# zfw1226/active_tracking_rl

Hardware: AMD Instinct MI355X
Metric: env steps/sec, Track2D-BlockPartialPZR-v0 @4096 envs, 1/2/4/8 GPU (higher is better)
Workload: dtype u8 map bits / f64 reward -> f32 obs+reward; policy fp32

## Files before the change

### active_tracking_rl_amd/csrc/gemm_tn_hip.hip

```cpp
#include <hip/hip_runtime.h>
#include <stdint.h>
#include <stdlib.h>

#include "../../include/atr_policy.h"

namespace atr {

typedef float f32x16 __attribute__((ext_vector_type(16)));

#ifndef ATR_TN_DIRECT
#define ATR_TN_DIRECT 1
#endif
#ifndef ATR_TN_PROBE
#define ATR_TN_PROBE 0
#endif
constexpr int kTile = 128, kLd = 128;
constexpr int kGemmThreads = 256;
constexpr long long kSmallK = 20 * 1024 + 1;
constexpr int tn_wg_per_cu(int kc) { return kc == 32 ? 2 : kc == 24 ? 3 : 4; }
static thread_local int g_tn_corun = 0;
static int tn_kc(long long K)
{
    static const int forced = getenv("ATR_GEMM_TN_KC") ? atoi(getenv("ATR_GEMM_TN_KC")) : 0;
    if (forced == 16 || forced == 32) return forced;
    if (g_tn_corun) return 16;
    return K < kSmallK ? 16 : 32;
}
static int tn_wg_per_cu_now(int kc) { return g_tn_corun ? 1 : tn_wg_per_cu(kc); }
constexpr unsigned kCorunLdsPad = 50000;

template <int kKC> struct GemmLds { float a[2][kKC][kLd]; float b[2][kKC][kLd]; };

constexpr int kMaxProblems = 8;

struct TnProblem {
    const float *x1, *x2;
    float *partial;
    float *cs_partial;
    const float *row_scale;
    float *c;
    float *cs_out0, *cs_out1;
    long long rs_shift;
    long long ld1, ld2;
    int M, N;
    int tile_begin;
    int red_begin;
};

struct TnGroup {
    TnProblem p[kMaxProblems];
    long long K;
    int count, slices, chunks_per_slice, tiles_total;
    int red_blocks;
};

#if ATR_TN_PROBE
__device__ unsigned long long g_tn_stamps[8192 * 4];
#endif

template <int kKC, bool kMixed>
__global__ __launch_bounds__(kGemmThreads, tn_wg_per_cu(kKC)) void k_gemm_tn(const TnGroup g)
{
    __shared__ __attribute__((aligned(16))) GemmLds<kKC> s;
    const int tid = (int)threadIdx.x, l = tid & 63, wave = tid >> 6;
#if ATR_TN_PROBE
    const unsigned long long st_rt = wall_clock64(), st_cy = __builtin_readcyclecounter();
#endif
    const int wm = wave >> 1, wn = wave & 1;
    const int i = (int)blockIdx.x, xcd = i & 7, in_xcd = i >> 3;
    const int slice = xcd + 8 * (in_xcd / g.tiles_total), tg = in_xcd % g.tiles_total;
    if (slice >= g.slices) return;
    int q = 0;
#pragma unroll
    for (int j = 1; j < kMaxProblems; j++)
        if (j < g.count && tg >= g.p[j].tile_begin) q = j;
    const float *__restrict__ x1 = g.p[q].x1, *__restrict__ x2 = g.p[q].x2;
    float *__restrict__ partial = g.p[q].partial, *__restrict__ colsum_partial = g.p[q].cs_partial;
    const float *__restrict__ row_scale = g.p[q].row_scale;
    const long long rs_shift = g.p[q].rs_shift, K = g.K;
    const int M = g.p[q].M, N = g.p[q].N, tile = tg - g.p[q].tile_begin, chunks_per_slice = g.chunks_per_slice;
    const int tiles_n = N / kTile;
    const int m0 = (tile / tiles_n) * kTile, n0 = (tile % tiles_n) * kTile;
    const long long k_begin = (long long)slice * chunks_per_slice * kKC;
    long long k_end = k_begin + (long long)chunks_per_slice * kKC;
    if (k_end > K) k_end = K;
    const int r = tid >> 5, c4 = tid & 31;
    const float4 *g1 = reinterpret_cast<const float4 *>(x1 + m0 + c4 * 4), *g2 = reinterpret_cast<const float4 *>(x2 + n0 + c4 * 4);
    const long long ldm = g.p[q].ld1 / 4, ldn = g.p[q].ld2 / 4;
    float4 ra0, ra1, rb0, rb1, ra2, ra3, rb2, rb3;
    float rs0 = 1.f, rs1 = 1.f, rs2 = 1.f, rs3 = 1.f;
    const bool do_colsum = colsum_partial != nullptr && n0 == 0;
    float cs = 0.f;
    const float4 zero4 = make_float4(0.f, 0.f, 0.f, 0.f);
#define GEMM_TN_FETCH(k0_)                                                     \
    {                                                                          \
        const long long ka_ = (k0_) + r, kb_ = (k0_) + r + 8, kc_ = (k0_) + r + 16, kd_ = (k0_) + r + 24;  \
        ra0 = zero4; ra1 = zero4; rb0 = zero4; rb1 = zero4; ra2 = zero4; ra3 = zero4; rb2 = zero4; rb3 = zero4; \
        if (ka_ < k_end) { ra0 = g1[ka_ * ldm]; rb0 = g2[ka_ * ldn]; }         \
        if (kb_ < k_end) { ra1 = g1[kb_ * ldm]; rb1 = g2[kb_ * ldn]; }         \
        if (kKC >= 24 && kc_ < k_end) { ra2 = g1[kc_ * ldm]; rb2 = g2[kc_ * ldn]; }         \
        if (kKC == 32 && kd_ < k_end) { ra3 = g1[kd_ * ldm]; rb3 = g2[kd_ * ldn]; }         \
        if (row_scale) {           \
            rs0 = 1.f; rs1 = 1.f; rs2 = 1.f; rs3 = 1.f;                       \
            if (ka_ >= rs_shift && ka_ < k_end) rs0 = row_scale[ka_ - rs_shift];                                       \
            if (kb_ >= rs_shift && kb_ < k_end) rs1 = row_scale[kb_ - rs_shift];                                       \
            if (kKC >= 24 && kc_ >= rs_shift && kc_ < k_end) rs2 = row_scale[kc_ - rs_shift];                         \
            if (kKC == 32 && kd_ >= rs_shift && kd_ < k_end) rs3 = row_scale[kd_ - rs_shift];                         \
        }                                                                      \
    }
#define GEMM_TN_STAGE(buf_)                                                    \
    {                                                                          \
        if (row_scale) {                                                       \
            ra0.x *= rs0; ra0.y *= rs0; ra0.z *= rs0; ra0.w *= rs0; ra1.x *= rs1; ra1.y *= rs1; ra1.z *= rs1; ra1.w *= rs1; \
            ra2.x *= rs2; ra2.y *= rs2; ra2.z *= rs2; ra2.w *= rs2; ra3.x *= rs3; ra3.y *= rs3; ra3.z *= rs3; ra3.w *= rs3; \
        }                                                                      \
        *reinterpret_cast<float4 *>(&s.a[buf_][r][c4 * 4]) = ra0;              \
        *reinterpret_cast<float4 *>(&s.a[buf_][r + 8][c4 * 4]) = ra1;          \
        *reinterpret_cast<float4 *>(&s.b[buf_][r][c4 * 4]) = rb0;              \
        *reinterpret_cast<float4 *>(&s.b[buf_][r + 8][c4 * 4]) = rb1;          \
        if (kKC >= 24) {                                                       \
        *reinterpret_cast<float4 *>(&s.a[buf_][(r + 16) % kKC][c4 * 4]) = ra2;         \
        *reinterpret_cast<float4 *>(&s.b[buf_][(r + 16) % kKC][c4 * 4]) = rb2;         \
        }                                                                      \
        if (kKC == 32) {                                                       \
        *reinterpret_cast<float4 *>(&s.a[buf_][(r + 24) % kKC][c4 * 4]) = ra3;         \
        *reinterpret_cast<float4 *>(&s.b[buf_][(r + 24) % kKC][c4 * 4]) = rb3;         \
        }                                                                      \
    }
    f32x16 acc00, acc01, acc10, acc11;
#pragma unroll
    for (int q = 0; q < 16; q++) { acc00[q] = 0.f; acc01[q] = 0.f; acc10[q] = 0.f; acc11[q] = 0.f; }
    const int kr = l >> 5, col = l & 31;
    auto compute = [&](int buf) {
        const float *pa = &s.a[buf][kr][wm * 64 + col], *pb = &s.b[buf][kr][wn * 64 + col];
        float a0 = pa[0], a1 = pa[32], b0 = pb[0], b1 = pb[32];
#pragma unroll
        for (int kp = 0; kp < kKC / 2; kp++) {
            float na0 = 0.f, na1 = 0.f, nb0 = 0.f, nb1 = 0.f;
            if (kp + 1 < kKC / 2) {
                na0 = pa[(kp + 1) * 2 * kLd]; na1 = pa[(kp + 1) * 2 * kLd + 32];
                nb0 = pb[(kp + 1) * 2 * kLd]; nb1 = pb[(kp + 1) * 2 * kLd + 32];
            }
            __builtin_amdgcn_sched_barrier(0);
            acc00 = __builtin_amdgcn_mfma_f32_32x32x2f32(a0, b0, acc00, 0, 0, 0);
            acc01 = __builtin_amdgcn_mfma_f32_32x32x2f32(a0, b1, acc01, 0, 0, 0);
            acc10 = __builtin_amdgcn_mfma_f32_32x32x2f32(a1, b0, acc10, 0, 0, 0);
            acc11 = __builtin_amdgcn_mfma_f32_32x32x2f32(a1, b1, acc11, 0, 0, 0);
            a0 = na0; a1 = na1; b0 = nb0; b1 = nb1;
        }
        if (do_colsum) {
            const float *pc = &s.a[buf][(tid >> 7) * (kKC / 2)][tid & 127];
#pragma unroll
            for (int q = 0; q < kKC / 2; q++) cs += pc[q * kLd];
        }
    };
    const bool direct = !kMixed || (kKC == 32 && ATR_TN_DIRECT && row_scale == nullptr && k_end > k_begin && (k_end - k_begin) % kKC == 0);
    if (direct) {
        auto dma = [&](long long k0, int buf) {
#pragma unroll
            for (int j = 0; j < kKC / 8; j++) {
                const long long kk = k0 + r + 8 * j;
                __builtin_amdgcn_global_load_lds((const __attribute__((address_space(1))) void *)(g1 + kk * ldm),
                                                 (__attribute__((address_space(3))) void *)(&s.a[buf][2 * wave + 8 * j][0]), 16, 0, 0);
                __builtin_amdgcn_global_load_lds((const __attribute__((address_space(1))) void *)(g2 + kk * ldn),
                                                 (__attribute__((address_space(3))) void *)(&s.b[buf][2 * wave + 8 * j][0]), 16, 0, 0);
            }
        };
        if (k_begin < k_end) dma(k_begin, 0);
        __builtin_amdgcn_s_waitcnt(0x0F70);
        __syncthreads();
        int buf = 0;
        for (long long k0 = k_begin; k0 < k_end; k0 += kKC, buf ^= 1) {
            if (k0 + kKC < k_end) dma(k0 + kKC, buf ^ 1);
            compute(buf);
            __builtin_amdgcn_s_waitcnt(0x0F70);
            __syncthreads();
        }
    } else if (kMixed) {
        GEMM_TN_FETCH(k_begin);
        GEMM_TN_STAGE(0);
        __syncthreads();
        int buf = 0;
        for (long long k0 = k_begin; k0 < k_end; k0 += kKC, buf ^= 1) {
            const bool more = k0 + kKC < k_end;
            if (more) GEMM_TN_FETCH(k0 + kKC);
            compute(buf);
            if (more) GEMM_TN_STAGE(buf ^ 1);
            __syncthreads();
        }
    }
    if (do_colsum) {
        float *red = &s.a[0][0][0];
        if (tid >= 128) red[tid - 128] = cs;
        __syncthreads();
        if (tid < 128) colsum_partial[(size_t)slice * M + m0 + tid] = cs + red[tid];
    }
#undef GEMM_TN_FETCH
#undef GEMM_TN_STAGE
    float *out = partial + (size_t)slice * M * N;
    auto store = [&](const f32x16 &acc, int mt, int nt) {
#pragma unroll
        for (int q = 0; q < 16; q++) {
            const int row = (q & 3) + 8 * (q >> 2) + 4 * kr;
            __builtin_nontemporal_store(acc[q], &out[(size_t)(m0 + wm * 64 + mt * 32 + row) * N + n0 + wn * 64 + nt * 32 + col]);
        }
    };
    store(acc00, 0, 0); store(acc01, 0, 1); store(acc10, 1, 0); store(acc11, 1, 1);
#if ATR_TN_PROBE
    if (tid == 0 && blockIdx.x < 8192) {
        unsigned long long *o = &g_tn_stamps[(size_t)blockIdx.x * 4];
        o[0] = st_rt; o[1] = wall_clock64(); o[2] = __builtin_readcyclecounter() - st_cy;
        o[3] = (unsigned long long)__builtin_amdgcn_s_getreg(63492) | ((unsigned long long)__builtin_amdgcn_s_getreg(63508) << 32);
    }
#endif
}

__global__ __launch_bounds__(256) void k_gemm_tn_reduce(const TnGroup g)
{
    const int b = (int)blockIdx.x;
    if (b < g.red_blocks) {
        int q = 0;
#pragma unroll
        for (int j = 1; j < kMaxProblems; j++)
            if (j < g.count && b >= g.p[j].red_begin) q = j;
        const long long mn = (long long)g.p[q].M * g.p[q].N;
        const long long i = ((long long)(b - g.p[q].red_begin) * 256 + threadIdx.x) * 4;
        if (i >= mn) return;
        const float *__restrict__ partial = g.p[q].partial;
        float4 acc = *reinterpret_cast<const float4 *>(partial + i);
#pragma unroll 8
        for (int z = 1; z < g.slices; z++) {
            const float4 t = *reinterpret_cast<const float4 *>(partial + (size_t)z * mn + i);
            acc.x += t.x; acc.y += t.y; acc.z += t.z; acc.w += t.w;
        }
        *reinterpret_cast<float4 *>(g.p[q].c + i) = acc;
        return;
    }
    int cb = b - g.red_blocks;
    for (int q = 0; q < g.count; q++) {
        if (!g.p[q].cs_partial) continue;
        const int nb = g.p[q].M / 4;
        if (cb >= nb) { cb -= nb; continue; }
        const int col = cb * 4 + (int)(threadIdx.x >> 6), lane = (int)(threadIdx.x & 63u), M = g.p[q].M;
        const float *__restrict__ partial = g.p[q].cs_partial;
        float acc = 0.f;
        for (int z = lane; z < g.slices; z += 64) acc += partial[(size_t)z * M + col];
        for (int m = 32; m >= 1; m >>= 1) acc += __shfl_xor(acc, m, 64);
        if (lane == 0) {
            if (g.p[q].cs_out0) g.p[q].cs_out0[col] = acc;
            if (g.p[q].cs_out1) g.p[q].cs_out1[col] = acc;
        }
        return;
    }
}

struct TnPlan { int slices, chunks_per_slice; };

static TnPlan gemm_tn_plan(long long K, int tiles)
{
    const int kKC = tn_kc(K), kWgPerCu = tn_wg_per_cu_now(kKC);
    const long long chunks = (K + kKC - 1) / kKC;
    const double eff_pair = 0.85, eff_solo = 0.6;
    int best = 8;
    double best_cost = 1e30;
    static const int forced = getenv("ATR_GEMM_TN_SLICES") ? atoi(getenv("ATR_GEMM_TN_SLICES")) : 0;
    for (int s = 8; s <= 512; s += 8) {
        if (s > chunks && s > 8) break;
        const long long cps = (chunks + s - 1) / s, wgs = (long long)tiles * s;
        const double rows = (double)cps * kKC + 64.0;
        const long long round = 256 * kWgPerCu;
        const long long full = wgs / round, rem = wgs - full * round;
        double cost = (double)full * kWgPerCu * rows / eff_pair;
        if (rem > 256) cost += (double)((rem + 255) / 256) * rows / eff_pair;
        else if (rem > 0) cost += rows / eff_solo;
        if (cost < best_cost - 1e-9) { best_cost = cost; best = s; }
    }
    if (forced >= 8 && forced % 8 == 0 && forced <= chunks) best = forced;
    TnPlan p;
    p.chunks_per_slice = (int)((chunks + best - 1) / best);
    p.slices = best;
    return p;
}

static int group_tiles(const atr_gemm_tn_problem *pr, int count)
{
    int tiles = 0;
    for (int q = 0; q < count; q++) {
        if (!pr[q].x1 || !pr[q].x2 || !pr[q].c || pr[q].M <= 0 || pr[q].N <= 0 || pr[q].M % kTile || pr[q].N % kTile) return -1;
        if ((pr[q].ld1 && (pr[q].ld1 < pr[q].M || pr[q].ld1 % 4)) || (pr[q].ld2 && (pr[q].ld2 < pr[q].N || pr[q].ld2 % 4))) return -1;
        tiles += (pr[q].M / kTile) * (pr[q].N / kTile);
    }
    return tiles;
}

}

using namespace atr;

#if ATR_TN_PROBE
extern "C" int atr_tn_stamps(unsigned long long *host, int wgs)
{
    return (int)hipMemcpyFromSymbol(host, HIP_SYMBOL(g_tn_stamps), (size_t)wgs * 4 * sizeof(unsigned long long));
}
#endif

extern "C" long long atr_gemm_tn_grouped_workspace_floats(const atr_gemm_tn_problem *problems, int count, long long K)
{
    if (!problems || count < 1 || count > kMaxProblems || K <= 0) return -1;
    const int tiles = group_tiles(problems, count);
    if (tiles < 0) return -1;
    const int s = gemm_tn_plan(K, tiles).slices;
    long long total = 0;
    for (int q = 0; q < count; q++) total += (long long)s * problems[q].M * problems[q].N + (long long)s * problems[q].M;
    return total;
}

extern "C" int atr_gemm_tn_grouped(const atr_gemm_tn_problem *problems, int count, long long K, float *workspace, void *stream)
{
    if (!problems || !workspace || count < 1 || count > kMaxProblems || K <= 0) return -1;
    const int tiles = group_tiles(problems, count);
    if (tiles < 0) return -1;
    TnGroup g;
    const TnPlan plan = gemm_tn_plan(K, tiles);
    g.slices = plan.slices; g.chunks_per_slice = plan.chunks_per_slice;
    g.K = K; g.count = count; g.tiles_total = tiles;
    float *ws = workspace;
    int tile_begin = 0, red_begin = 0, cs_blocks = 0;
    for (int q = 0; q < kMaxProblems; q++) {
        TnProblem &d = g.p[q];
        if (q >= count) { d = g.p[0]; d.tile_begin = 1 << 30; d.red_begin = 1 << 30; continue; }
        const atr_gemm_tn_problem &p = problems[q];
        const long long mn = (long long)p.M * p.N;
        d.x1 = p.x1; d.x2 = p.x2; d.c = p.c; d.row_scale = p.row_scale; d.rs_shift = p.row_scale_shift; d.M = p.M; d.N = p.N;
        d.ld1 = p.ld1 ? p.ld1 : p.M; d.ld2 = p.ld2 ? p.ld2 : p.N;
        d.cs_out0 = p.colsum0; d.cs_out1 = p.colsum1;
        d.partial = ws; ws += (size_t)g.slices * mn;
        const bool cs = p.colsum0 || p.colsum1;
        d.cs_partial = cs ? ws : nullptr;
        if (cs) { ws += (size_t)g.slices * p.M; cs_blocks += p.M / 4; }
        d.tile_begin = tile_begin; tile_begin += (p.M / kTile) * (p.N / kTile);
        d.red_begin = red_begin; red_begin += (int)((mn / 4 + 255) / 256);
    }
    g.red_blocks = red_begin;
    hipStream_t st = (hipStream_t)stream;
    const dim3 grid((unsigned)(g.slices * tiles)), block(kGemmThreads);
    const int kc = tn_kc(K);
    static const unsigned forced_pad = getenv("ATR_GEMM_TN_LDS_PAD") ? (unsigned)atoi(getenv("ATR_GEMM_TN_LDS_PAD")) : 0u;
    const unsigned lds_pad = forced_pad ? forced_pad : (g_tn_corun && kc == 16 ? kCorunLdsPad : 0u);
    static bool attr_set = false;
    if (lds_pad && !attr_set) {
        const int lim = 96 * 1024;
        if (hipFuncSetAttribute((const void *)k_gemm_tn<16, false>, hipFuncAttributeMaxDynamicSharedMemorySize, lim) != hipSuccess ||
            hipFuncSetAttribute((const void *)k_gemm_tn<16, true>, hipFuncAttributeMaxDynamicSharedMemorySize, lim) != hipSuccess ||
            hipFuncSetAttribute((const void *)k_gemm_tn<32, false>, hipFuncAttributeMaxDynamicSharedMemorySize, lim) != hipSuccess ||
            hipFuncSetAttribute((const void *)k_gemm_tn<32, true>, hipFuncAttributeMaxDynamicSharedMemorySize, lim) != hipSuccess)
            return -2;
        attr_set = true;
    }
    bool all_direct = ATR_TN_DIRECT && K % kc == 0;
    for (int q = 0; q < count; q++) all_direct = all_direct && problems[q].row_scale == nullptr;
    if (kc == 16) {
        if (all_direct) hipLaunchKernelGGL((k_gemm_tn<16, false>), grid, block, lds_pad, st, g);
        else hipLaunchKernelGGL((k_gemm_tn<16, true>), grid, block, lds_pad, st, g);
    } else {
        if (all_direct) hipLaunchKernelGGL((k_gemm_tn<32, false>), grid, block, lds_pad, st, g);
        else hipLaunchKernelGGL((k_gemm_tn<32, true>), grid, block, lds_pad, st, g);
    }
    hipLaunchKernelGGL(k_gemm_tn_reduce, dim3((unsigned)(red_begin + cs_blocks)), dim3(256), 0, st, g);
    return hipGetLastError() == hipSuccess ? 0 : -2;
}

extern "C" int atr_gemm_tn_set_corun(int on)
{
    const int was = g_tn_corun;
    g_tn_corun = on ? 1 : 0;
    return was;
}

extern "C" long long atr_gemm_tn_workspace_floats(long long K, int M, int N)
{
    atr_gemm_tn_problem p = {};
    float dummy = 0.f;
    p.x1 = p.x2 = &dummy; p.c = &dummy; p.M = M; p.N = N; p.colsum0 = &dummy;
    return atr_gemm_tn_grouped_workspace_floats(&p, 1, K);
}

extern "C" int atr_gemm_tn(const float *x1, const float *x2, float *c, float *workspace, long long K, int M, int N,
                           const float *row_scale, float *colsum, void *stream)
{
    atr_gemm_tn_problem p = {};
    p.x1 = x1; p.x2 = x2; p.c = c; p.M = M; p.N = N; p.row_scale = row_scale; p.row_scale_shift = 0; p.colsum0 = colsum;
    return atr_gemm_tn_grouped(&p, 1, K, workspace, stream);
}
```

### active_tracking_rl_amd/fused.py

```python
import ctypes as C
import json
import os
import re
import sys

import torch

from . import vec_env

_lib = None


class ActStepArgs(C.Structure):
    _fields_ = [("ig", C.c_void_p * 2), ("hg", C.c_void_p * 2), ("bias", C.c_void_p * 2), ("c_prev", C.c_void_p * 2),
                ("h_out", C.c_void_p * 2), ("c_out", C.c_void_p * 2), ("acts", C.c_void_p * 2),
                ("actor_w", C.c_void_p * 2), ("actor_b", C.c_void_p * 2), ("emb", C.c_void_p), ("done_prev", C.c_void_p),
                ("actions_out", C.c_void_p), ("counter", C.c_void_p), ("seed", C.c_ulonglong), ("ordinal", C.c_uint),
                ("A", C.c_int), ("N", C.c_int), ("R", C.c_int), ("hm_out", C.c_void_p * 2), ("hm_ld", C.c_longlong)]


class CoopStepArgs(C.Structure):
    _fields_ = [("y", C.c_void_p * 2), ("fc_w", C.c_void_p * 2), ("fc_b", C.c_void_p * 2), ("w_cat", C.c_void_p * 2),
                ("ldy", C.c_longlong * 2), ("kfc", C.c_int * 2), ("fh", C.c_void_p), ("gates", C.c_void_p),
                ("fh_pstride", C.c_longlong), ("fh_ld", C.c_longlong), ("F", C.c_int), ("workgroups", C.c_int),
# ... 1224 lines not shown


@torch.no_grad()
def gae_returns(rewards, values, notdone, gamma, tau):
    T, N, A = rewards.shape[0], rewards.shape[1], rewards.shape[2]
    rewards, values, notdone = rewards.contiguous(), values.contiguous(), notdone.contiguous()
    ret, gae = torch.empty_like(rewards), torch.empty_like(rewards)
    lib().atr_gae_returns(_p(rewards), _p(values), _p(notdone), float(gamma), float(tau), _p(ret), _p(gae),
                          T, N, A, _stream(rewards))
    return ret, gae


def _col_stride(t):
    return t.shape[-2] if t.shape[-1] == 1 else t.shape[-1]


@torch.no_grad()
def heads_values(h, critic, values, off):
    h = h.contiguous()
    rows, R = h.shape
    A = _col_stride(values)
    lib().atr_heads_values(_p(h), _p(critic.weight), _p(critic.bias), _p(values), rows, R, A, off, _stream(h))


@torch.no_grad()
def heads_values2(hs, critics, values):
    h0, h1 = hs[0].contiguous(), hs[1].contiguous()
    rows, R = h0.shape
    assert h1.shape == h0.shape
    A = _col_stride(values)
    lib().atr_heads_values2(_p(h0), _p(critics[0].weight), _p(critics[0].bias), 0, _p(h1), _p(critics[1].weight),
                            _p(critics[1].bias), 1, _p(values), rows, R, A, _stream(h0))


def _act_layout(actions, rows):
    if actions.dim() == 2 and actions.stride(1) == 1 and actions.shape[0] * actions.shape[1] == rows:
        return actions, actions.shape[1], actions.stride(0)
    a = actions.reshape(rows).contiguous()
    return a, rows, 0


def _head_grads(dh, gs, A, R, has_aux):
    o = (A + 2) * R
    dwa, dwc, dwx = gs[:A * R].view(A, R), gs[A * R:(A + 1) * R].view(1, R), gs[(A + 1) * R:o].view(1, R)
    dba, dbc, dbx = gs[o:o + A], gs[o + A:o + A + 1], gs[o + A + 1:o + A + 2]
    return [dh, dwa, dba, dwc, dbc, dwx if has_aux else None, dbx if has_aux else None]


class _HeadsLossPair(torch.autograd.Function):

    @staticmethod
    def forward(ctx, cfg, *t):
        L = lib()
        arr = (HeadsLossArgs * 2)()
        hs, keep = [], []
        for p in range(2):
            h, wa, ba, wc, bc, waux, baux = t[7 * p:7 * p + 7]
            c = cfg[p]
            h = h.contiguous()
            rows, R = h.shape
            A = wa.shape[0]
            rec = (A + 2) * R + (A + 2) + 4
            dh = torch.empty_like(h)
            gs = torch.empty(rec + 1, dtype=torch.float32, device=h.device)
            ws = torch.empty(L.atr_heads_workspace_floats(rows, R, A), dtype=torch.float32, device=h.device)
            acts, act_n, act_ts = _act_layout(c["actions"], rows)
            ret = c["ret"]
            a = arr[p]
            a.h, a.actions, a.act_n, a.act_tstride = h.data_ptr(), acts.data_ptr(), act_n, act_ts
            a.ret, a.gae, a.val = ret.data_ptr(), c["gae"].data_ptr(), c["val"].data_ptr()
            a.stride = _col_stride(ret)
            a.off = c["off"]
            r_aux = c.get("r_aux")
            a.r_aux = r_aux.data_ptr() if r_aux is not None else None
            a.aux_stride = _col_stride(r_aux) if r_aux is not None else 0
            a.aux_off = c.get("aux_off", 0)
            a.wa, a.ba, a.wc = wa.data_ptr(), ba.data_ptr(), wc.data_ptr()
            a.waux = waux.data_ptr() if waux is not None else None
            a.baux = baux.data_ptr() if baux is not None else None
            a.scale, a.scale_aux, a.w_ent = float(c["scale"]), float(c["scale_aux"]), float(c["w_ent"])
            a.dh, a.grads_and_sums, a.workspace = dh.data_ptr(), gs.data_ptr(), ws.data_ptr()
            a.rows, a.R, a.A = rows, R, A
            hs.append((dh, gs, A, R, waux is not None, rec))
            keep += [h, acts, ws]
        stats = torch.empty((2, 4), dtype=torch.float32, device=hs[0][0].device)
        arr[0].stats_out, arr[1].stats_out = stats.data_ptr(), stats.data_ptr() + 16
        L.atr_heads_loss_multi(arr, 2, float(cfg[0]["stats_scale"]), _stream(hs[0][0]))
        ctx.save_for_backward(hs[0][0], hs[0][1], hs[1][0], hs[1][1])
        ctx.dims = [(x[2], x[3], x[4]) for x in hs]
        ctx.set_materialize_grads(False)
        ctx.mark_non_differentiable(stats)
        return hs[0][1][hs[0][5]], hs[1][1][hs[1][5]], stats

    @staticmethod
    def backward(ctx, g0, g1, gstats):
        sv = ctx.saved_tensors
        out = [None]
        for p in range(2):
            if (g0, g1)[p] is None:
                out += [None] * 7
            else:
                out += _head_grads(sv[2 * p], sv[2 * p + 1], *ctx.dims[p])
        return tuple(out)


def heads_loss_pair(hs, actors, critics, auxes, cfg):
    t = []
    for p in range(2):
        aux = auxes[p]
        t += [hs[p], actors[p].weight, actors[p].bias, critics[p].weight, critics[p].bias,
              aux.weight if aux is not None else None, aux.bias if aux is not None else None]
    return _HeadsLossPair.apply(cfg, *t)


class _HeadsLoss(torch.autograd.Function):

    @staticmethod
    def forward(ctx, h, wa, ba, wc, bc, waux, baux, actions, ret, gae, val, off, r_aux, aux_off, scale, scale_aux, w_ent,
                unit_coeff=False):
        L = lib()
        h = h.contiguous()
        rows, R = h.shape
        A = wa.shape[0]
        stride = _col_stride(ret)
        rec = (A + 2) * R + (A + 2) + 4
        dh = torch.empty_like(h)
        gs = torch.empty(rec + 1, dtype=torch.float32, device=h.device)
        ws = torch.empty(L.atr_heads_workspace_floats(rows, R, A), dtype=torch.float32, device=h.device)
        actions = actions.contiguous()
        aux_stride = _col_stride(r_aux) if r_aux is not None else 0
        L.atr_heads_loss(_p(h), _p(actions), _p(ret), _p(gae), _p(val), stride, off, _pn(r_aux), aux_stride, aux_off,
                         _p(wa), _p(ba), _p(wc), _pn(waux), _pn(baux), float(scale), float(scale_aux), float(w_ent),
                         _p(dh), _p(gs), _p(ws), rows, R, A, _stream(h))
        ctx.save_for_backward(dh, gs)
        ctx.dims = (A, R, waux is not None)
        ctx.unit_coeff = bool(unit_coeff)
        stats = gs[rec - 4:rec]
        ctx.mark_non_differentiable(stats)
        return gs[rec], stats

    @staticmethod
    def backward(ctx, gloss, gstats):
        dh, gs = ctx.saved_tensors
        if not ctx.unit_coeff:
            dh, gs = dh * gloss, gs * gloss
        return tuple(_head_grads(dh, gs, *ctx.dims)) + (None,) * 11


def heads_loss(h, actor, critic, aux, actions, ret, gae, val, off, r_aux, aux_off, scale, scale_aux, w_ent,
               unit_coeff=False):
    return _HeadsLoss.apply(h, actor.weight, actor.bias, critic.weight, critic.bias,
                            aux.weight if aux is not None else None, aux.bias if aux is not None else None,
                            actions, ret, gae, val, off, r_aux, aux_off, scale, scale_aux, w_ent, unit_coeff)


class _EmbedAdd(torch.autograd.Function):

    @staticmethod
    def forward(ctx, f, w, b, actions):
        if not (f.stride(1) == 1 and f.stride(0) >= f.shape[1] and f.stride(0) % 4 == 0):
            f = f.contiguous()
        rows, Cc = f.shape
        A = w.shape[1]
        wc, bc = w.contiguous(), b.contiguous()
        out = torch.empty((rows, Cc), dtype=f.dtype, device=f.device)
        acts, act_n, act_ts = _act_layout(actions, rows)
        lib().atr_embed_add_ld(_p(f), f.stride(0), _p(wc), _p(bc), _p(acts), 1, act_n, act_ts, _p(out), rows, Cc, A,
                               _stream(f))
        ctx.save_for_backward(acts)
        ctx.dims = (Cc, A, act_n, act_ts)
        return out

    @staticmethod
    def backward(ctx, dout):
        (acts,) = ctx.saved_tensors
        Cc, A, act_n, act_ts = ctx.dims
        dout = dout.contiguous()
        rows = dout.shape[0]
        L = lib()
        ws = torch.empty(L.atr_embed_grad_workspace_floats(rows, Cc, A), dtype=torch.float32, device=dout.device)
        dw = torch.empty((Cc, A), dtype=torch.float32, device=dout.device)
        db = torch.empty(Cc, dtype=torch.float32, device=dout.device)
        L.atr_embed_grad(_p(dout), _p(acts), 1, act_n, act_ts, _p(dw), _p(db), _p(ws), rows, Cc, A, _stream(dout))
        return dout, dw, db, None


def embed_add(f, linear, actions):
    assert actions.dtype == torch.int64 and f.dim() == 2 and actions.numel() == f.shape[0]
    return _EmbedAdd.apply(f, linear.weight, linear.bias, actions)


use_gemm_tn = True
use_grouped_dw = True
_deferred = None


class DeferredWeightGrads(object):

    MAX = 8

    def __init__(self, bucket):
        self.views = {}
        for prm, v in zip(bucket.params, bucket.grad_views()):
            self.views[prm.data_ptr()] = v
        self.problems, self.K, self.registered = [], None, set()
        self.after = []

    def view(self, prm):
        return self.views.get(prm.data_ptr()) if prm is not None else None

    def _problem(self, x1, x2, weight, biases=(), row_scale=None, shift=0, rows=None):
        K, M = x1.shape
        N = x2.shape[1]
        whole = self.view(weight)
        bw = [self.view(b) for b in biases]
        if whole is None or any(v is None for v in bw) or len(bw) > 2:
            return None
        dst, bv = whole, bw
        if rows is not None:
            if whole.dim() != 2 or not (0 <= rows[0] < rows[1] <= whole.shape[0]):
                return None
            dst, bv = whole[rows[0]:rows[1]], [v[rows[0]:rows[1]] for v in bw]
        if ((self.K is not None and K != self.K) or K < 4096 or M % 128 or N % 128
                or not (x1.is_cuda and x1.dtype == torch.float32 and x2.dtype == torch.float32
                        and x1.stride(1) == 1 and x1.stride(0) >= M and x1.stride(0) % 4 == 0 and x1.data_ptr() % 16 == 0
                        and x2.stride(1) == 1 and x2.stride(0) >= N and x2.stride(0) % 4 == 0
                        and x2.data_ptr() % 16 == 0)
                or tuple(dst.shape) != (M, N) or any(tuple(v.shape) != (M,) for v in bv)
                or (row_scale is not None and not row_scale.is_contiguous())):
            return None
        return (x1, x2, dst, row_scale, int(shift), bv, M, N), (whole, bw)

    def _commit(self, rec):
        prob, (whole, bw) = rec
        self.K = prob[0].shape[0]
        self.problems.append(prob)
        self.registered.update(v.data_ptr() for v in [whole] + bw)
        return whole, bw

    def add(self, x1, x2, weight, biases=(), row_scale=None, shift=0, rows=None):
        if len(self.problems) >= self.MAX:
            return None
        rec = self._problem(x1, x2, weight, biases, row_scale, shift, rows)
        return self._commit(rec) if rec is not None else None

    def add_all(self, products):
        if len(self.problems) + len(products) > self.MAX:
            return None
        recs = [self._problem(**kw) for kw in products]
        if any(rec is None for rec in recs) or len(set(rec[0][0].shape[0] for rec in recs)) > 1:
            return None
        return [self._commit(rec) for rec in recs]

    def check(self, grads):
        got = set(g.data_ptr() for g in grads if g is not None)
        if not self.registered <= got:
            raise RuntimeError("grouped weight gradients: autograd did not return the registered bucket slices as they are "
                               "(a parameter with more than one gradient contribution?); set fused.use_grouped_dw = False")

    @torch.no_grad()
    def flush(self):
        if not self.problems:
            return
        n = len(self.problems)
        arr = (GemmTnProblem * n)()
        for q, (x1, x2, dst, rs, shift, bv, M, N) in enumerate(self.problems):
            arr[q].x1, arr[q].x2, arr[q].c = x1.data_ptr(), x2.data_ptr(), dst.data_ptr()
            arr[q].row_scale = rs.data_ptr() if rs is not None else None
            arr[q].row_scale_shift = shift
            arr[q].colsum0 = bv[0].data_ptr() if len(bv) > 0 else None
            arr[q].colsum1 = bv[1].data_ptr() if len(bv) > 1 else None
            arr[q].M, arr[q].N = M, N
            arr[q].ld1, arr[q].ld2 = x1.stride(0), x2.stride(0)
        L = lib()
        x0 = self.problems[0][0]
        ws = torch.empty(L.atr_gemm_tn_grouped_workspace_floats(arr, n, self.K), dtype=torch.float32, device=x0.device)
        L.atr_gemm_tn_grouped(arr, n, self.K, _p(ws), _stream(x0))
        self.problems, self.K = [], None
        for fn in self.after:
            fn()
        self.after = []


class deferred_weight_grads(object):

    def __init__(self, bucket):
        self.bucket = bucket

    def __enter__(self):
        global _deferred
        self.q = DeferredWeightGrads(self.bucket) if (use_grouped_dw and use_gemm_tn and self.bucket.grad.is_cuda) else None
        _deferred = self.q
        return self.q

    def __exit__(self, *exc):
        global _deferred
        _deferred = None
        return False



class gemm_tn_corun(object):

    def __init__(self, on=True):
        self.on, self.was = bool(on), None

    def __enter__(self):
        self.was = lib().atr_gemm_tn_set_corun(1 if self.on else 0)
        return self

    def __exit__(self, *exc):
        lib().atr_gemm_tn_set_corun(self.was)
        return False


@torch.no_grad()
def gemm_tn(x1, x2, row_scale=None, colsum=False):
    K, M = x1.shape
    N = x2.shape[1]
    if (use_gemm_tn and x1.is_cuda and x1.dtype == torch.float32 and x2.dtype == torch.float32 and M % 128 == 0
            and N % 128 == 0 and K >= 4096 and x1.is_contiguous() and x2.is_contiguous()):
        L = lib()
        ws = torch.empty(L.atr_gemm_tn_workspace_floats(K, M, N), dtype=torch.float32, device=x1.device)
        c = torch.empty((M, N), dtype=torch.float32, device=x1.device)
        cs = torch.empty(M, dtype=torch.float32, device=x1.device) if colsum else None
        rs = row_scale.contiguous() if row_scale is not None else None
        L.atr_gemm_tn(_p(x1), _p(x2), _p(c), _p(ws), K, M, N, _pn(rs), _pn(cs), _stream(x1))
        return (c, cs) if colsum else c
    if row_scale is not None:
        x1 = x1 * row_scale.unsqueeze(1)
    c = x1.t() @ x2
    return (c, x1.sum(0)) if colsum else c


def rollout_consts_ok(consts):
    ts = []
    for l in consts["lstm"]:
        ts += [l.weight_ih, l.weight_hh, l.bias_ih, l.bias_hh]
    if "fa" in consts:
        ts += [consts["fa"].weight, consts["fa"].bias]
    return all(t.is_cuda and t.is_contiguous() and t.dtype == torch.float32 and t.data_ptr() % 16 == 0 for t in ts)


@torch.no_grad()
def rollout_begin(hxs, cxs, h_all, c_all, obs_src=None, obs_dst=None, consts=None, counter=None):
    N, A, R = hxs.shape
    assert hxs.is_contiguous() and cxs.is_contiguous() and h_all.is_contiguous() and c_all.is_contiguous()
    assert h_all.shape[0] == A and h_all.shape[2] == N and h_all.shape[3] == R and hxs.dtype == torch.float32
    nbytes = 0
    if obs_src is not None:
        assert obs_src.is_contiguous() and obs_dst.is_contiguous()
        nbytes = obs_src.numel() * obs_src.element_size()
        assert nbytes == obs_dst.numel() * obs_dst.element_size() and nbytes % 4 == 0
    if consts is None:
        lib().atr_rollout_begin(_p(hxs), _p(cxs), _p(h_all), _p(c_all), h_all.stride(0), _pn(obs_src), _pn(obs_dst), nbytes,
                                N, A, R, _stream(hxs))
        return
    k = RolloutConsts()
    for p, l in enumerate(consts["lstm"]):
        k.w_ih[p], k.w_hh[p] = l.weight_ih.data_ptr(), l.weight_hh.data_ptr()
        k.b_ih[p], k.b_hh[p] = l.bias_ih.data_ptr(), l.bias_hh.data_ptr()
    k.bsum = consts["bsum"].data_ptr()
    k.F = int(consts["F"])
    if "w_cat" in consts:
        k.w_cat = consts["w_cat"].data_ptr()
        fh = consts["fh_all"]
        k.fh0, k.fh_pstride, k.fh_ld = fh.data_ptr(), fh.stride(0), fh.stride(2)
    if "emb_ih" in consts:
        fa = consts["fa"]
        k.fa_w, k.fa_b, k.emb_ih, k.A_act = fa.weight.data_ptr(), fa.bias.data_ptr(), consts["emb_ih"].data_ptr(), fa.weight.shape[1]
    if counter is not None:
        k.counter = counter.data_ptr()
    lib().atr_rollout_begin2(_p(hxs), _p(cxs), _p(h_all), _p(c_all), h_all.stride(0), _pn(obs_src), _pn(obs_dst), nbytes,
                              N, A, R, C.byref(k), _stream(hxs))


@torch.no_grad()
def rollout_end(h_all, c_all, dones, hxs, cxs, eps_len, keep, obs_src=None, obs_dst=None, done_dst=None):
    A, T1, N, R = h_all.shape
    T = T1 - 1
    assert dones.shape == (T, N) and dones.dtype == torch.uint8 and dones.is_contiguous()
    assert hxs.shape == (N, A, R) and hxs.is_contiguous() and cxs.is_contiguous() and keep.is_contiguous()
    assert eps_len.dtype == torch.int32 and eps_len.is_contiguous() and keep.shape == (T, N)
    nbytes = 0
    if obs_src is not None:
        assert obs_src.is_contiguous() and obs_dst.is_contiguous() and obs_src.dtype == obs_dst.dtype
        nbytes = obs_src.numel() * obs_src.element_size()
        assert nbytes == obs_dst.numel() * obs_dst.element_size() and nbytes % 4 == 0
    if done_dst is not None:
        assert done_dst.dtype == torch.uint8 and done_dst.is_contiguous() and done_dst.numel() == N
    lib().atr_rollout_end2(_p(h_all[0, T]), _p(c_all[0, T]), h_all.stride(0), _p(dones), _p(hxs), _p(cxs), _p(eps_len),
                           _p(keep), T, N, A, R, _pn(obs_src), _pn(obs_dst), nbytes, _pn(done_dst), _stream(hxs))


@torch.no_grad()
def adam_step(p, grad, exp_avg, exp_avg_sq, max_exp_avg_sq, scalars, step_size, lr, beta1, beta2, eps, weight_decay,
              torch_eps=False):
    lib().atr_adam_step(_p(p), _p(grad), _p(exp_avg), _p(exp_avg_sq), _pn(max_exp_avg_sq), _p(scalars), _p(step_size),
                        float(lr), float(beta1), float(beta2), float(eps), float(weight_decay), 1 if torch_eps else 0,
                        p.numel(), _stream(p))


@torch.no_grad()
def rmsprop_step(p, grad, square_avg, lr, alpha, eps, weight_decay):
    lib().atr_rmsprop_step(_p(p), _p(grad), _p(square_avg), float(lr), float(alpha), float(eps), float(weight_decay),
                           p.numel(), _stream(p))
```

Measured before the change: 17.46 million.

## Add deeper multi-stage LDS pipeline options for co-run TN weight-gradient GEMM

Adds a configurable co-run form (K-chunk size and stage count) for the TN GEMM used when it runs concurrently with other work. The direct global-to-LDS path gets a 3- or 4-stage ring buffer with partial vmcnt waits, so loads run further ahead of compute. LDS is allocated dynamically when it exceeds the static limit. The slice-planning efficiency constant is changed for co-run. The default form is 16x2, which matches the old two-stage behaviour, so deeper staging only applies when selected by environment variable or argument. The main default change is the LDS padding total and the planning efficiency constant.

```diff
diff --git a/active_tracking_rl_amd/csrc/gemm_tn_hip.hip b/active_tracking_rl_amd/csrc/gemm_tn_hip.hip
--- a/active_tracking_rl_amd/csrc/gemm_tn_hip.hip
+++ b/active_tracking_rl_amd/csrc/gemm_tn_hip.hip
@@ -1,5 +1,6 @@
 #include <hip/hip_runtime.h>
 #include <stdint.h>
+#include <stdio.h>
 #include <stdlib.h>
 
 #include "../../include/atr_policy.h"
@@ -19,17 +20,36 @@
 constexpr long long kSmallK = 20 * 1024 + 1;
 constexpr int tn_wg_per_cu(int kc) { return kc == 32 ? 2 : kc == 24 ? 3 : 4; }
 static thread_local int g_tn_corun = 0;
+struct TnCorun { int kc, stages; };
+constexpr int kCorunDefault = 162;
+static bool tn_corun_code_ok(int code) { return code == 162 || code == 164 || code == 322 || code == 323; }
+static int tn_corun_default()
+{
+    static const int code = [] {
+        const char *e = getenv("ATR_GEMM_TN_CORUN");
+        int kc = 0, st = 0;
+        if (e && sscanf(e, "%dx%d", &kc, &st) == 2 && tn_corun_code_ok(kc * 10 + st)) return kc * 10 + st;
+        return kCorunDefault;
+    }();
+    return code;
+}
+static TnCorun tn_corun_form() { return TnCorun{g_tn_corun / 10, g_tn_corun % 10}; }
+static int tn_kc_forced()
+{
+    static const int forced = getenv("ATR_GEMM_TN_KC") ? atoi(getenv("ATR_GEMM_TN_KC")) : 0;
+    return forced == 16 || forced == 32 ? forced : 0;
+}
 static int tn_kc(long long K)
 {
-    static const int forced = getenv("ATR_GEMM_TN_KC") ? atoi(getenv("ATR_GEMM_TN_KC")) : 0;
-    if (forced == 16 || forced == 32) return forced;
-    if (g_tn_corun) return 16;
+    if (tn_kc_forced()) return tn_kc_forced();
+    if (g_tn_corun) return tn_corun_form().kc;
     return K < kSmallK ? 16 : 32;
 }
 static int tn_wg_per_cu_now(int kc) { return g_tn_corun ? 1 : tn_wg_per_cu(kc); }
-constexpr unsigned kCorunLdsPad = 50000;
-
-template <int kKC> struct GemmLds { float a[2][kKC][kLd]; float b[2][kKC][kLd]; };
+constexpr unsigned kCorunLdsTotal = 32768 + 50000;
+
+template <int kKC, int kStages> struct GemmLds { float a[kStages][kKC][kLd]; float b[kStages][kKC][kLd]; };
+constexpr bool tn_lds_dynamic(int kc, int stages) { return 2 * stages * kc * kLd * 4 > 64 * 1024; }
 
 constexpr int kMaxProblems = 8;
 
@@ -58,10 +78,19 @@
 __device__ unsigned long long g_tn_stamps[8192 * 4];
 #endif
 
-template <int kKC, bool kMixed>
-__global__ __launch_bounds__(kGemmThreads, tn_wg_per_cu(kKC)) void k_gemm_tn(const TnGroup g)
-{
-    __shared__ __attribute__((aligned(16))) GemmLds<kKC> s;
+template <int kKC, bool kMixed, int kStages = 2>
+__global__ __launch_bounds__(kGemmThreads, kStages == 2 ? tn_wg_per_cu(kKC) : 1) void k_gemm_tn(const TnGroup g)
+{
+    static_assert(kStages == 2 || !kMixed, "the register-staged path keeps two buffers");
+    GemmLds<kKC, kStages> *lds;
+    if constexpr (tn_lds_dynamic(kKC, kStages)) {
+        extern __shared__ __attribute__((aligned(16))) unsigned char tn_dynamic_lds[];
+        lds = reinterpret_cast<GemmLds<kKC, kStages> *>(tn_dynamic_lds);
+    } else {
+        __shared__ __attribute__((aligned(16))) GemmLds<kKC, kStages> tn_static_lds;
+        lds = &tn_static_lds;
+    }
+    GemmLds<kKC, kStages> &s = *lds;
     const int tid = (int)threadIdx.x, l = tid & 63, wave = tid >> 6;
 #if ATR_TN_PROBE
     const unsigned long long st_rt = wall_clock64(), st_cy = __builtin_readcyclecounter();
@@ -166,6 +195,7 @@
                                                  (__attribute__((address_space(3))) void *)(&s.b[buf][2 * wave + 8 * j][0]), 16, 0, 0);
             }
         };
+        if constexpr (kStages == 2) {
         if (k_begin < k_end) dma(k_begin, 0);
         __builtin_amdgcn_s_waitcnt(0x0F70);
         __syncthreads();
@@ -175,6 +205,28 @@
             compute(buf);
             __builtin_amdgcn_s_waitcnt(0x0F70);
             __syncthreads();
+        }
+        } else {
+            constexpr int kLoads = 2 * (kKC / 8);
+            static_assert((kStages - 2) * kLoads == 8, "the partial wait below is vmcnt(8)");
+            const int n = k_begin < k_end ? (int)((k_end - k_begin) / kKC) : 0;
+#pragma unroll
+            for (int j = 0; j < kStages - 1; j++)
+                if (j < n) dma(k_begin + (long long)j * kKC, j);
+            if (n >= kStages - 1) __builtin_amdgcn_s_waitcnt(0x0078);
+            else __builtin_amdgcn_s_waitcnt(0x0070);
+            __builtin_amdgcn_s_barrier();
+            int slot = 0, fill = kStages - 1;
+            for (int c = 0; c < n; c++) {
+                const bool ahead = c + kStages - 1 < n;
+                if (ahead) dma(k_begin + (long long)(c + kStages - 1) * kKC, fill);
+                compute(slot);
+                if (ahead) __builtin_amdgcn_s_waitcnt(0x0078);
+                else __builtin_amdgcn_s_waitcnt(0x0070);
+                __builtin_amdgcn_s_barrier();
+                slot = slot + 1 == kStages ? 0 : slot + 1;
+                fill = fill + 1 == kStages ? 0 : fill + 1;
+            }
         }
     } else if (kMixed) {
         GEMM_TN_FETCH(k_begin);
@@ -255,12 +307,13 @@
 }
 
 struct TnPlan { int slices, chunks_per_slice; };
+constexpr double kEffCorun = 0.67;
 
 static TnPlan gemm_tn_plan(long long K, int tiles)
 {
     const int kKC = tn_kc(K), kWgPerCu = tn_wg_per_cu_now(kKC);
     const long long chunks = (K + kKC - 1) / kKC;
-    const double eff_pair = 0.85, eff_solo = 0.6;
+    const double eff_pair = g_tn_corun ? kEffCorun : 0.85, eff_solo = g_tn_corun ? kEffCorun : 0.6;
     int best = 8;
     double best_cost = 1e30;
     static const int forced = getenv("ATR_GEMM_TN_SLICES") ? atoi(getenv("ATR_GEMM_TN_SLICES")) : 0;
@@ -344,26 +397,39 @@
     g.red_blocks = red_begin;
     hipStream_t st = (hipStream_t)stream;
     const dim3 grid((unsigned)(g.slices * tiles)), block(kGemmThreads);
-    const int kc = tn_kc(K);
+    int kc = tn_kc(K), stages = 2;
+    bool all_direct = ATR_TN_DIRECT && K % kc == 0;
+    for (int q = 0; q < count; q++) all_direct = all_direct && problems[q].row_scale == nullptr;
+    const bool corun = g_tn_corun && !tn_kc_forced();
+    if (corun && all_direct) stages = tn_corun_form().stages;
+    if (corun && !all_direct && kc != 16) {
+        g.chunks_per_slice *= kc / 16;
+        kc = 16;
+    }
     static const unsigned forced_pad = getenv("ATR_GEMM_TN_LDS_PAD") ? (unsigned)atoi(getenv("ATR_GEMM_TN_LDS_PAD")) : 0u;
-    const unsigned lds_pad = forced_pad ? forced_pad : (g_tn_corun && kc == 16 ? kCorunLdsPad : 0u);
+    const unsigned lds_bytes = 2u * (unsigned)(stages * kc) * kLd * sizeof(float);
+    const bool dynamic = tn_lds_dynamic(kc, stages);
+    unsigned lds_pad = forced_pad ? forced_pad : (g_tn_corun && (corun || kc == 16) ? kCorunLdsTotal - lds_bytes : 0u);
+    if (dynamic) lds_pad = lds_bytes;
     static bool attr_set = false;
     if (lds_pad && !attr_set) {
         const int lim = 96 * 1024;
         if (hipFuncSetAttribute((const void *)k_gemm_tn<16, false>, hipFuncAttributeMaxDynamicSharedMemorySize, lim) != hipSuccess ||
             hipFuncSetAttribute((const void *)k_gemm_tn<16, true>, hipFuncAttributeMaxDynamicSharedMemorySize, lim) != hipSuccess ||
             hipFuncSetAttribute((const void *)k_gemm_tn<32, false>, hipFuncAttributeMaxDynamicSharedMemorySize, lim) != hipSuccess ||
-            hipFuncSetAttribute((const void *)k_gemm_tn<32, true>, hipFuncAttributeMaxDynamicSharedMemorySize, lim) != hipSuccess)
+            hipFuncSetAttribute((const void *)k_gemm_tn<32, true>, hipFuncAttributeMaxDynamicSharedMemorySize, lim) != hipSuccess ||
+            hipFuncSetAttribute((const void *)k_gemm_tn<16, false, 4>, hipFuncAttributeMaxDynamicSharedMemorySize, lim) != hipSuccess ||
+            hipFuncSetAttribute((const void *)k_gemm_tn<32, false, 3>, hipFuncAttributeMaxDynamicSharedMemorySize, lim) != hipSuccess)
             return -2;
         attr_set = true;
     }
-    bool all_direct = ATR_TN_DIRECT && K % kc == 0;
-    for (int q = 0; q < count; q++) all_direct = all_direct && problems[q].row_scale == nullptr;
     if (kc == 16) {
-        if (all_direct) hipLaunchKernelGGL((k_gemm_tn<16, false>), grid, block, lds_pad, st, g);
+        if (all_direct && stages == 4) hipLaunchKernelGGL((k_gemm_tn<16, false, 4>), grid, block, lds_pad, st, g);
+        else if (all_direct) hipLaunchKernelGGL((k_gemm_tn<16, false>), grid, block, lds_pad, st, g);
         else hipLaunchKernelGGL((k_gemm_tn<16, true>), grid, block, lds_pad, st, g);
     } else {
-        if (all_direct) hipLaunchKernelGGL((k_gemm_tn<32, false>), grid, block, lds_pad, st, g);
+        if (all_direct && stages == 3) hipLaunchKernelGGL((k_gemm_tn<32, false, 3>), grid, block, lds_pad, st, g);
+        else if (all_direct) hipLaunchKernelGGL((k_gemm_tn<32, false>), grid, block, lds_pad, st, g);
         else hipLaunchKernelGGL((k_gemm_tn<32, true>), grid, block, lds_pad, st, g);
     }
     hipLaunchKernelGGL(k_gemm_tn_reduce, dim3((unsigned)(red_begin + cs_blocks)), dim3(256), 0, st, g);
@@ -373,7 +439,7 @@
 extern "C" int atr_gemm_tn_set_corun(int on)
 {
     const int was = g_tn_corun;
-    g_tn_corun = on ? 1 : 0;
+    g_tn_corun = on == 0 ? 0 : tn_corun_code_ok(on) ? on : tn_corun_default();
     return was;
 }
 
diff --git a/active_tracking_rl_amd/fused.py b/active_tracking_rl_amd/fused.py
--- a/active_tracking_rl_amd/fused.py
+++ b/active_tracking_rl_amd/fused.py
@@ -1550,11 +1550,14 @@
 
 class gemm_tn_corun(object):
 
-    def __init__(self, on=True):
+    FORMS = {"16x2": 162, "16x4": 164, "32x2": 322, "32x3": 323}
+
+    def __init__(self, on=True, form=None):
         self.on, self.was = bool(on), None
+        self.code = 1 if form is None else self.FORMS[form]
 
     def __enter__(self):
-        self.was = lib().atr_gemm_tn_set_corun(1 if self.on else 0)
+        self.was = lib().atr_gemm_tn_set_corun(self.code if self.on else 0)
         return self
 
     def __exit__(self, *exc):
```

Result: no change. 17.33 million (-0.7%).
